# tool-recommender-bot/logparser

Measured on AMD Instinct MI355X. Metric: GB/s (and lines/s) of 'combined' log parsed per GPU and per 8xMI355X node, higher is better.
Workload: dtype u8

## Files before the change

logparser_amd/csrc/kernels_common.h:

```cpp
#pragma once
#include <hip/hip_runtime.h>

#ifndef LP_KERNEL_TU
#define LP_KERNEL_TU 1
#endif

#include <algorithm>

#include "kernels.h"
#include "lp_device.h"

namespace lp {
namespace {

constexpr int CHUNK = 64 * 1024;
constexpr int NL_THREADS = 256;
constexpr int PW = 64;

typedef uint32_t u32x4 __attribute__((ext_vector_type(4)));

__device__ __forceinline__ uint32_t byte_eq(uint32_t w, uint32_t c4) {
    uint32_t x = w ^ c4;
    return ~(((x & 0x7F7F7F7Fu) + 0x7F7F7F7Fu) | x | 0x7F7F7F7Fu);
}
__device__ __forceinline__ uint32_t bits16(uint32_t m0, uint32_t m1, uint32_t m2, uint32_t m3) {
    return bcls::nib(m0) | (bcls::nib(m1) << 4) | (bcls::nib(m2) << 8) | (bcls::nib(m3) << 12);
}

__device__ __forceinline__ uint32_t term_bits(uint4 v, const uint8_t* p, uint64_t pos, uint64_t nbytes) {
    uint32_t lf = bits16(byte_eq(v.x, 0x0A0A0A0Au), byte_eq(v.y, 0x0A0A0A0Au), byte_eq(v.z, 0x0A0A0A0Au),
                         byte_eq(v.w, 0x0A0A0A0Au));
    uint32_t cr = bits16(byte_eq(v.x, 0x0D0D0D0Du), byte_eq(v.y, 0x0D0D0D0Du), byte_eq(v.z, 0x0D0D0D0Du),
                         byte_eq(v.w, 0x0D0D0D0Du));
    if (pos + 16 > nbytes) {
        const uint32_t live = nbytes > pos ? (1u << (uint32_t)(nbytes - pos)) - 1u : 0u;
        lf &= live;
        cr &= live;
    }
    if (cr) {
        uint32_t next_lf = lf >> 1;
        if ((cr & 0x8000u) && pos + 16 < nbytes && p[pos + 16] == '\n') next_lf |= 0x8000u;
        cr &= ~next_lf;
    }
    return lf | cr;
}
__device__ __forceinline__ uint32_t term16(const uint8_t* p, uint64_t pos, uint64_t nbytes) {
    uint4 v = make_uint4(0, 0, 0, 0);
    if (pos + 16 <= nbytes && ((uintptr_t)(p + pos) & 15) == 0) {
        v = *reinterpret_cast<const uint4*>(p + pos);
    } else {
        uint32_t w[4] = {0, 0, 0, 0};
        for (uint64_t k = pos; k < pos + 16 && k < nbytes; ++k) w[(k - pos) >> 2] |= (uint32_t)p[k] << (8 * ((k - pos) & 3));
        v = make_uint4(w[0], w[1], w[2], w[3]);
    }
    return term_bits(v, p, pos, nbytes);
}

__device__ __forceinline__ int lane_id() {
    return (int)__builtin_amdgcn_mbcnt_hi(~0u, __builtin_amdgcn_mbcnt_lo(~0u, 0u));
}

struct WaveStack {
    uint32_t* base;
    __device__ uint32_t& operator[](int k) const { return base[k * PW]; }
};

template <typename LN>
__device__ __forceinline__ LN owner_line(const LN& L, int own) {
    LN R = L;
    R.o = (uint32_t)__shfl((int)L.o, own);
    R.n = __shfl(L.n, own);
    if constexpr (!LN::has_masks)
        R.b = reinterpret_cast<decltype(L.b)>(__shfl((unsigned long long)(uintptr_t)L.b, own));
    return R;
}

struct WaveLines {
    int64_t li0, li, lend;
    bool active;
    uint64_t s, e, w0, w1;
    int n;
};
__device__ __forceinline__ WaveLines wave_lines(const Columns& C, int64_t wave, int64_t n_lines, uint64_t nbytes) {
    WaveLines W;
    W.li0 = wave * PW;
    W.li = W.li0 + (int64_t)lane_id();
    W.active = W.li < n_lines;
    W.lend = W.li0 + PW < n_lines ? W.li0 + PW : n_lines;
    W.s = W.e = 0;
    if (W.active) {
        W.s = C.line_off[W.li];
        W.e = C.line_off[W.li + 1] - 1;
    }
    W.n = (int)((W.e - W.s) > (uint64_t)0x7FFFFFFF ? 0x7FFFFFFF : (W.e - W.s));
    W.w0 = C.line_off[W.li0] & ~15ull;
    W.w1 = C.line_off[W.lend];
    if (W.w1 > nbytes) W.w1 = nbytes;
    return W;
}

__device__ __forceinline__ int crlf_len(int n, uint32_t last) { return n - (n > 0 && last == '\r' ? 1 : 0); }
__device__ __forceinline__ int crlf_len_hbm(const uint8_t* buf, const WaveLines& W) {
    return W.active ? crlf_len(W.n, W.n > 0 ? buf[W.e - 1] : 0u) : W.n;
}

__device__ __forceinline__ bool stage_window(const uint8_t* __restrict__ buf, uint64_t nbytes, uint64_t w0, uint64_t w1,
                                             uint8_t* win, uint16_t* msk16) {
    const int lane = lane_id();
    const int nv = (int)((w1 - w0 + 15) >> 4);
    const int nv4 = (nv + 3) & ~3;
    uint32_t bad = 0;
    constexpr int SB = 20;
    const uint64_t full_end = nbytes & ~15ull;
    for (int k0 = lane; k0 < nv4; k0 += SB * PW) {
        u32x4 v[SB];
#pragma unroll
        for (int j = 0; j < SB; ++j) {
            const int k = k0 + j * PW;
            const uint64_t p = w0 + 16ull * k;
            v[j] = u32x4{0, 0, 0, 0};
            if (k < nv && p + 16 <= full_end) v[j] = __builtin_nontemporal_load(reinterpret_cast<const u32x4*>(buf + p));
        }
#pragma unroll
        for (int j = 0; j < SB; ++j) {
            const int k = k0 + j * PW;
            if (k >= nv4) continue;
            const uint64_t p = w0 + 16ull * k;
            if (k < nv && p + 16 > full_end) {
                auto word = [&](uint64_t q) {
                    uint32_t w = 0;
#pragma unroll
                    for (int b = 0; b < 4; ++b) w |= q + b < nbytes ? (uint32_t)buf[q + b] << (8 * b) : 0u;
                    return w;
                };
                v[j] = u32x4{word(p), word(p + 4), word(p + 8), word(p + 12)};
            }
            *reinterpret_cast<u32x4*>(win + 16 * k) = v[j];
            uint32_t m0, m1, g = 0, lf, other, cr;
            bcls::classify16p(v[j][0], v[j][1], v[j][2], v[j][3], m0, m1, g, lf, other);
            if (other) bcls::classify16c(v[j][0], v[j][1], v[j][2], v[j][3], g, cr);
            if (k < nv) bad |= g;
            msk16[8 * (k >> 2) + (k & 3)] = (uint16_t)m0;
            msk16[8 * (k >> 2) + 4 + (k & 3)] = (uint16_t)m1;
        }
    }
    return !__any(bad != 0);
}

struct WaveCounts {
    uint32_t act = 0, ok = 0, bad = 0, written = 0;
    uint32_t gathered = 0;
    __device__ __forceinline__ void store(LP_G uint32_t* wave_counts, int64_t wave) const {
        if (lane_id() == 0) {
            uint4 c, d;
            c.x = act;
            c.y = ok;
            c.z = bad;
            c.w = act - ok - bad;
            d.x = written;
            d.y = gathered;
            d.z = d.w = 0;
            uint4* wc = reinterpret_cast<uint4*>(wave_counts + WC_WORDS * (size_t)wave);
            wc[0] = c;
            wc[1] = d;
        }
    }
    __device__ __forceinline__ void store(const Columns& C, int64_t wave) const { store(C.wave_counts, wave); }
};

template <bool MULTI, typename LN>
__device__ __forceinline__ void parse_wave(const Program& P, const Elem* elems, const Columns& C, const LN& L,
                                           bool active, int64_t li, WaveStack stk, bool clean, WaveCounts& WC) {
    LineOut o;
    o.status = ST_OK;
    LP_PROF(1);
    if (active) phase1<MULTI>(P, elems, L, o, stk, C, li, clean, P.n_fmt > 1 ? (int)C.fmt_id[li] : 0);
    LP_PROF(9);
    if (active) write_line(P, o, C, li);
    if (active && !P.has_phase2()) C.arena_base[li] = 0;
    WC.act += (uint32_t)__popcll(__ballot(active));
    WC.ok += (uint32_t)__popcll(__ballot(active && o.status == ST_OK));
    WC.bad += (uint32_t)__popcll(__ballot(active && o.status == ST_BAD));
}

__device__ __forceinline__ u32x4 load16(const uint8_t* __restrict__ buf, uint64_t nbytes, uint64_t p) {
    if (p + 16 <= nbytes) return *reinterpret_cast<const u32x4*>(buf + p);
    uint32_t w[4] = {0, 0, 0, 0};
    for (int c = 0; c < 16; ++c) w[c >> 2] |= p + c < nbytes ? (uint32_t)buf[p + c] << (8 * (c & 3)) : 0u;
    return u32x4{w[0], w[1], w[2], w[3]};
}

__device__ __forceinline__ void load_elems(const Program& P, Elem* s_elems) {
    for (int k = lane_id(); k < P.n_elems; k += PW) s_elems[k] = P.elems[k];
}

__device__ __forceinline__ uint32_t select64(uint64_t m, uint32_t k) {
    uint32_t pos = 0, v = (uint32_t)m, c = (uint32_t)__popc(v);
    if (k >= c) { k -= c; v = (uint32_t)(m >> 32); pos = 32; }
    c = (uint32_t)__popc(v & 0xFFFFu);
    if (k >= c) { k -= c; v >>= 16; pos += 16; }
    c = (uint32_t)__popc(v & 0xFFu);
    if (k >= c) { k -= c; v >>= 8; pos += 8; }
    c = (uint32_t)__popc(v & 0xFu);
    if (k >= c) { k -= c; v >>= 4; pos += 4; }
    c = (uint32_t)__popc(v & 3u);
    if (k >= c) { k -= c; v >>= 2; pos += 2; }
    return pos + (k >= (v & 1u) ? 1u : 0u);
}
__device__ __forceinline__ int lsb64(uint64_t m) { return (int)__builtin_ctzll(m); }
__device__ __forceinline__ int msb64(uint64_t m) { return 63 - (int)__builtin_clzll(m); }

template <typename T>
__device__ __forceinline__ T wave_incl_scan(T x) {
    const int lane = lane_id();
    for (int d = 1; d < 64; d <<= 1) {
        const T y = __shfl_up(x, d);
        if (lane >= d) x += y;
    }
    return x;
}
template <typename T>
__device__ __forceinline__ T wave_sum(T x) {
    for (int d = 32; d > 0; d >>= 1) x += __shfl_xor(x, d);
    return x;
}

}
}
```

logparser_amd/csrc/uri.hip:

```cpp
#include "kernels_common.h"

namespace lp {

namespace {

constexpr uint32_t URI_CAP = 8512;
#ifndef LP_URI_QR
#define LP_URI_QR 4
#endif
#ifndef LP_URI_GR
#define LP_URI_GR 9
#endif

template <int NU>
struct UriLane {
    bool ok;
    int fmt;
    uint64_t ls;
    RegArr<NU> sp, cs, usep;
};

template <int NU>
__device__ __forceinline__ UriLane<NU> uri_lane(const Program& P, const Columns& C, int64_t li, bool active) {
    UriLane<NU> U;
    U.sp.fill(0);
    U.cs.fill(0);
    U.usep.fill(0);
    U.ok = false;
    U.fmt = 0;
    U.ls = 0;
    if (!active) return U;
    const uint8_t st = C.status[li];
    const int fmt = P.n_fmt > 1 ? (int)C.fmt_id[li] : 0;
    U.ls = C.line_off[li];
    const uint32_t tf = C.tok_flags[li];
    uint32_t raw[NU], kind[NU];
    for (int u = 0; u < NU; ++u) {
        raw[u] = 0;
        kind[u] = FL_FULL;
        if (u >= P.n_uri || P.uri[u].src_q >= 0) continue;
        if (P.uri[u].src_tok >= 0) {
            raw[u] = C.tok_span[P.uri[u].src_tok][li];
            kind[u] = (tf >> P.uri[u].src_tok) & 1u ? FL_NONE : FL_FULL;
        } else {
            raw[u] = C.fl_uri[P.uri[u].src_fl][li];
            kind[u] = C.fl_kind[P.uri[u].src_fl][li];
        }
    }
    U.ok = st == ST_OK;
    U.fmt = U.ok ? fmt : 0;
    if (U.ok)
        for (int u = 0; u < P.n_uri && u < NU; ++u) {
            const int a = (int)(raw[u] & 0xFFFF), b = (int)(raw[u] >> 16);
            if (P.uri[u].fmt == U.fmt && P.uri[u].src_q < 0 && kind[u] != FL_NONE && b > a) U.sp.set(u, mkspan(a, b));
        }
    return U;
}


template <bool SLOT, typename CL>
__device__ __forceinline__ void uri_walk_coop(const Program& P, int u, const CL& L, bool part, int a, int b,
                                              uint32_t usep, const Arena& A, UriWalk& Wk) {
    const int lane = lane_id();
    const bool table = u >= 0 && P.uri[u].want_query && P.uri[u].query_stage >= 0;
    const uint32_t cnt = part ? usep : 0u;
    uint32_t x = cnt;
    for (int d = 1; d < 64; d <<= 1) {
        const uint32_t y = __shfl_up(x, d);
        if (lane >= d) x += y;
    }
    const uint32_t eb = x - cnt, E = __shfl(x, 63);
    const uint32_t tab = (A.used + 15) & ~15u;
    const unsigned long long reg = (unsigned long long)(uintptr_t)A.p;
    int resume = -1, fa = -1, fpct = -1, lastB = -1, lastPP = -1;
    uint32_t count = 0;
    bool rw = false;
    for (uint32_t g0 = 0; g0 < E; g0 += PW) {
        const uint32_t g = g0 + (uint32_t)lane;
        const bool valid = g < E;
        int ow = 0;
        for (int st = 32; st; st >>= 1)
            if (__shfl((int)eb, ow + st) <= (int)g) ow += st;
        const uint32_t ebo = (uint32_t)__shfl((int)eb, ow);
        const uint32_t oo = (uint32_t)__shfl((int)L.o, ow);
        const int oa = __shfl(a, ow), ob = __shfl(b, ow);
        uint32_t Aq = 0;
        if (valid) {
            const uint32_t A0 = oo + (uint32_t)oa, A1 = oo + (uint32_t)ob, WL = (A1 - 1) >> 6;
            uint32_t W = A0 >> 6, k = g - ebo;
            uint64_t m = L.mask(MC_UEV, W) & (~0ull << (A0 & 63));
            for (;;) {
                if (W == WL) m &= ~0ull >> (63 - ((A1 - 1) & 63));
                const uint32_t c = (uint32_t)__popcll(m);
                if (k < c || W >= WL) break;
                k -= c;
                ++W;
                m = L.mask(MC_UEV, W);
            }
            Aq = (W << 6) + select64(m, k);
        }
        const int q = (int)(Aq - oo);
        CL Lo = L;
        Lo.o = oo;
        Lo.n = ob;
        const uint32_t w = valid ? load_u32_at(Lo, q) : 0u;
        const uint32_t c = w & 0xFFu;
        const bool pct = c == '%';
        const bool bad_pct = pct && (q + 2 >= ob || !is_hex((w >> 8) & 0xFFu) || !is_hex((w >> 16) & 0xFFu));
        const bool stop = valid && (c == '#' || c == ';' || c >= 0x80 || bad_pct);
        const bool aq = c == '&' || c == '?';
        const int cres = __shfl(resume, ow), cfa = __shfl(fa, ow), clB = __shfl(lastB, ow), clPP = __shfl(lastPP, ow);
        const uint32_t ccount = (uint32_t)__shfl((int)count, ow);
        const int s0 = (int)ebo - (int)g0;
        const uint64_t below = (1ull << lane) - 1ull;
        const uint64_t seg_lt = valid ? below & (~0ull << (s0 > 0 ? s0 : 0)) : 0ull;
        const uint64_t Bstop = __ballot(stop);
        const bool live = valid && !stop && cres < 0 && !(Bstop & seg_lt);
        const uint64_t Baq = __ballot(live && aq);
        const uint64_t mfa = Baq & seg_lt;
        const int qfa = __shfl(q, mfa ? lsb64(mfa) : lane);
        const int fa_j = cfa >= 0 ? cfa : (mfa ? qfa : -1);
        const bool pp = live && ((pct && !bad_pct) || c == '+');
        const bool otable = SLOT ? __shfl((int)table, ow) != 0 : table;
        const bool isB = otable && live && aq && fa_j >= 0;
        const uint64_t BB = __ballot(isB), BPP = __ballot(pp);
        const uint64_t mB = BB & seg_lt, mP = BPP & seg_lt;
        const int qpb = __shfl(q, mB ? msb64(mB) : lane), qpp = __shfl(q, mP ? msb64(mP) : lane);
        const bool first_piece = !mB && clB < 0;
        const int pb = mB ? qpb : (clB >= 0 ? clB : fa_j);
        const int lpp = mP ? qpp : clPP;
        const int lp = first_piece ? lpp : (lpp > pb ? lpp : -1);
        const bool emit = isB && q > pb + 1;
        const uint64_t BE = __ballot(emit);
        const bool rwj = live && fa_j >= 0 && ((aq && c == '?') || (!aq && !pct && uri_needs_encode(c)));
        const uint64_t BR = __ballot(rwj);
        const unsigned long long oreg = __shfl(reg, ow);
        const uint32_t otab = (uint32_t)__shfl((int)tab, ow);
        if (emit) {
            const uint32_t idx = ccount + (uint32_t)__popcll(BE & seg_lt);
            const uint64_t t0 = (uint64_t)(uint32_t)(pb + 1) | ((uint64_t)(uint32_t)q << 16) | ((uint64_t)(uint32_t)(lp + 1) << 48);
            *reinterpret_cast<LP_G u32x4*>(reinterpret_cast<LP_G uint8_t*>(oreg) + otab + 16 * idx) =
                u32x4{(uint32_t)t0, (uint32_t)(t0 >> 32), 0u, 0u};
        }
        const int so = (int)eb - (int)g0, eo = (int)(eb + cnt) - (int)g0;
        const int so_c = so < 0 ? 0 : so > PW ? PW : so, eo_c = eo < 0 ? 0 : eo > PW ? PW : eo;
        const uint64_t segm = so_c < eo_c ? ((eo_c == PW ? ~0ull : (1ull << eo_c) - 1ull) & (~0ull << so_c)) : 0ull;
        const uint64_t ms = Bstop & segm, mf = Baq & segm, mpct = __ballot(live && pct) & segm, mb = BB & segm,
                       mpp = BPP & segm;
        const int q_s = __shfl(q, ms ? lsb64(ms) : lane), q_f = __shfl(q, mf ? lsb64(mf) : lane);
        const int q_p = __shfl(q, mpct ? lsb64(mpct) : lane), q_b = __shfl(q, mb ? msb64(mb) : lane);
        const int q_pp = __shfl(q, mpp ? msb64(mpp) : lane);
        if (resume < 0 && ms) resume = q_s;
        if (fa < 0 && mf) fa = q_f;
        if (fpct < 0 && mpct) fpct = q_p;
        if (mb) lastB = q_b;
        if (mpp) lastPP = q_pp;
        count += (uint32_t)__popcll(BE & segm);
        rw = rw || (BR & segm) != 0;
    }
    if (!part) return;
    Wk.resume = resume;
    Wk.fa = fa;
    Wk.first_pct = fpct;
    Wk.rewr = rw ? 2u : 0u;
    QueryTable& T = Wk.T;
    if (table && fa >= 0) {
        T.on = T.set = true;
        T.maxp = usep + 1;
        T.tab = tab;
        T.reg = tab + 16 * T.maxp;
        T.s = (lastB >= 0 ? lastB : fa) + 1;
        T.count = count;
        T.lp = lastB >= 0 ? (lastPP > lastB ? lastPP : -1) : lastPP;
    } else {
        T.lp = lastPP;
    }
}

template <int NU, int NQ, bool COOP, bool SLOT, bool QUEUE, typename LU, typename LL>
__device__ __forceinline__ void uri_wave(const Program& P, const Columns& C, UriLane<NU>& U, LU&& lu, LL&& ll,
                                         bool active, int64_t li, int64_t wave, WaveCounts& WC, bool& redo) {
    const int lane = lane_id();
    const int nq = P.n_query < NQ ? P.n_query : NQ;
    uint32_t need = 0;
    if (U.ok)
        for (int u = 0; u < P.n_uri && u < NU; ++u) {
            const uint32_t s = U.sp.get(u);
            if (!s) continue;
            uint32_t ev;
            need += uri_need(P, u, lu(u), (int)(s & 0xFFFF), (int)(s >> 16), ev);
            U.usep.set(u, ev);
        }
    int lend = 0;
    if (U.ok) {
        for (int j = 0; j < P.n_list; ++j)
            if (P.list[j].fmt == U.fmt) lend = max(lend, (int)(C.tok_span[P.list[j].tok][li] >> 16));
        for (int j = 0; j < P.n_pair; ++j)
            if (P.pair[j].fmt == U.fmt) lend = max(lend, (int)(C.tok_span[P.pair[j].tok][li] >> 16));
    }
    if (lend) ll(lend, [&](const auto& LH) { need += list_need(P, U.fmt, LH, C, li) + pair_need(P, U.fmt, LH, C, li); });
    need = (need + 15) & ~15u;
    uint32_t x = need;
    for (int d = 1; d < 64; d <<= 1) {
        uint32_t y = __shfl_up(x, d);
        if (lane >= d) x += y;
    }
    const uint32_t total = __shfl(x, 63);
    const int shard = (int)(wave % ARENA_SHARDS);
    unsigned long long wbase = 0;
    if (lane == 63 && total) wbase = atomicAdd(&C.meta->shard_top[16 * shard], (unsigned long long)total + 12ull);
    wbase = (__shfl(wbase, 63) + 15) & ~15ull;
    const bool fits = wbase + total <= C.shard_cap;
    LP_PROF(26);
    uint32_t written = 0;
    unsigned long long my_region = 0;
    UriOutT<NQ> o;
    o.qlist.fill(0);
    o.qpend.fill(0);
    o.status = U.ok ? ST_OK : ST_BAD;
    Arena A{C.arena, 0, 0};
    bool live = false;
    if (U.ok) {
        if (!fits && need) {
            o.status = ST_FALLBACK;
            atomicAdd(&C.meta->arena_ovf, 1ull);
        } else {
            const unsigned long long mine = (unsigned long long)shard * C.shard_cap + wbase + x - need;
            my_region = mine;
            C.arena_base[li] = mine;
            A = Arena{C.arena + mine, 0, need};
            A.top = &C.meta->shard_top[16 * shard];
            A.base = wbase + x - need;
            A.limit = C.shard_cap;
            live = true;
        }
    }
    const int nu = P.n_uri < NU ? P.n_uri : NU;
    for (int sl = 0; sl < nu; ++sl) {
        int u = sl;
        if constexpr (SLOT) {
            u = -1;
            for (int v = 0, c = 0; v < nu; ++v)
                if (P.uri[v].fmt == U.fmt) {
                    if (c == sl) u = v;
                    ++c;
                }
            if (!__any(u >= 0)) break;
        }
        const bool fmt_ok = live && o.status == ST_OK && u >= 0 && P.uri[u].fmt == U.fmt;
        const uint32_t sp = U.sp.get(u);
        const int a = (int)(sp & 0xFFFF), b = (int)(sp >> 16);
        const bool part = fmt_ok && b > a;
        if (fmt_ok && !part) {
            C.u_flags[u][li] = 0;
            if (P.uri[u].query_stage >= 0) { C.q_count[P.uri[u].query_stage][li] = 0; C.q_params[P.uri[u].query_stage][li] = 0; }
        }
        LP_PROF(10 + 2 * sl);
        UriWalk Wk;
        if constexpr (COOP) {
            LP_PROF(50 + 4 * sl);
            uri_walk_coop<SLOT>(P, u, lu(u), part, a, b, U.usep.get(u), A, Wk);
            LP_PROF(51 + 4 * sl);
        } else if (part) {
            uri_walk_fast(P, u, lu(u), a, b, U.usep.get(u), A, Wk);
        }
        if (part) {
            const int st = uri_stage_rest<UR_OFF>(P, u, lu(u), a, b, U.usep.get(u), A, C, li, o, Wk);
            if (st != ST_OK) o.status = st;
        }
        LP_PROF(11 + 2 * sl);
    }
    if (live && lend && o.status == ST_OK) {
        bool filled = true;
        ll(lend, [&](const auto& LH) { filled = list_fill(P, U.fmt, LH, A, C, li) && pair_fill(P, U.fmt, LH, A, C, li); });
        if (!filled) o.status = ST_FALLBACK;
    }
    if (live) {
        if (A.ovf) {
            o.status = ST_FALLBACK;
            atomicAdd(&C.meta->arena_ovf, 1ull);
        }
        written = A.used - A.slack + A.extra;
    }
    LP_PROF(21);
    if (nq > 0) {
        constexpr int QR = LP_URI_QR;
        __syncthreads();
        const bool has = U.ok && o.status == ST_OK && need != 0;
        const unsigned long long my_ab = has ? my_region : 0ull;
        uint64_t piece_ovf = 0;
        uint32_t np = 0;
        for (int qs = 0; qs < nq; ++qs) np += has ? o.qpend.get(qs) : 0u;
        uint32_t incl = np;
        for (int d = 1; d < 64; d <<= 1) {
            const uint32_t y = __shfl_up(incl, d);
            if (lane >= d) incl += y;
        }
        const uint32_t base = incl - np, tot = __shfl(incl, 63);
        auto piece = [&](int ow, uint32_t j, int& pq, uint32_t& soff) {
            uint32_t cum = 0;
            pq = 0;
            soff = 0;
            for (int qs = 0; qs < nq; ++qs) {
                const uint32_t c = (uint32_t)__shfl((int)(has ? o.qpend.get(qs) : 0u), ow);
                const uint32_t l = (uint32_t)__shfl((int)o.qlist.get(qs), ow);
                if (j >= cum && j < cum + c) {
                    pq = qs;
                    soff = l + 16 * (j - cum);
                }
                cum += c;
            }
        };
        auto owner_view = [&](int ow, int pq) {
            auto OL = owner_line(lu(P.query[0].uri), ow);
            for (int qs = 1; qs < nq; ++qs) {
                const auto V = owner_line(lu(P.query[qs].uri), ow);
                if (pq == qs) OL = V;
            }
            return OL;
        };
        for (uint32_t g0 = 0; g0 < tot; g0 += QR * PW) {
            int own[QR], pqs[QR];
            uint32_t soffs[QR];
            uint64_t t0[QR];
#pragma unroll
            for (int k = 0; k < QR; ++k) {
                own[k] = 0;
                pqs[k] = 0;
                soffs[k] = 0;
                t0[k] = 0;
                if (g0 + (uint32_t)(k * PW) >= tot) continue;
                const uint32_t g = g0 + (uint32_t)(k * PW + lane);
                int ow = 0;
                for (int st = 32; st; st >>= 1)
                    if (__shfl(base, ow + st) <= g) ow += st;
                own[k] = ow;
                const uint32_t ob = __shfl(base, ow);
                const unsigned long long oab = __shfl(my_ab, ow);
                piece(ow, g - ob, pqs[k], soffs[k]);
                if (g < tot) t0[k] = *reinterpret_cast<const LP_G uint64_t*>(C.arena + oab + soffs[k]);
            }
            LP_PROF(17);
            QPrep qp[QR];
            uint32_t mine = 0;
#pragma unroll
            for (int k = 0; k < QR; ++k) {
                if (g0 + (uint32_t)(k * PW) >= tot) continue;
                const uint32_t g = g0 + (uint32_t)(k * PW + lane);
                const auto OL = owner_view(own[k], pqs[k]);
                if (g < tot) qp[k] = query_prep(OL, t0[k]);
                mine += qp[k].need;
            }
            LP_PROF(18);
            uint32_t x = mine;
            for (int d = 1; d < 64; d <<= 1) {
                const uint32_t y = __shfl_up(x, d);
                if (lane >= d) x += y;
            }
            const uint32_t rtot = __shfl(x, 63);
            unsigned long long rbase = 0;
            if (lane == 63 && rtot) rbase = atomicAdd(&C.meta->shard_top[16 * shard], (unsigned long long)rtot);
            unsigned long long at = __shfl(rbase, 63) + x - mine;
            LP_PROF(19);
#pragma unroll
            for (int k = 0; k < QR; ++k) {
                if (g0 + (uint32_t)(k * PW) >= tot) continue;
                const uint32_t g = g0 + (uint32_t)(k * PW + lane);
                const int ow = own[k];
                const unsigned long long oab = __shfl(my_ab, ow);
                const auto OL = owner_view(ow, pqs[k]);
                bool povf = false;
                if (g < tot) {
                    LP_G uint64_t* slot = reinterpret_cast<LP_G uint64_t*>(C.arena + oab + soffs[k]);
                    const unsigned long long rel = oab - (unsigned long long)shard * C.shard_cap;
                    if (qp[k].need && (at + qp[k].need > C.shard_cap || at - rel + qp[k].need > 0x7FFFFFFFull)) {
                        slot[0] = REF_SKIP;
                        slot[1] = 0;
                        povf = true;
                        atomicAdd(&C.meta->arena_ovf, 1ull);
                    } else {
                        Arena A{C.arena + oab, (uint32_t)(at - rel), (uint32_t)(at - rel + qp[k].need)};
                        written += query_finish(P, P.query[pqs[k]], OL, A, C.arena + oab, slot, qp[k]);
                    }
                    at += qp[k].need;
                }
                for (uint64_t m = __ballot(povf); m; m &= m - 1) piece_ovf |= 1ull << __shfl(ow, (int)__builtin_ctzll(m));
            }
        }
        if (((piece_ovf >> lane) & 1) && o.status == ST_OK) o.status = ST_FALLBACK;
    }
    LP_PROF(22);
    redo = false;
    if (U.ok && o.status == ST_REPAIR) {
        o.status = ST_FALLBACK;
        if constexpr (QUEUE) {
            const unsigned long long k = atomicAdd(&C.meta->uri_fix_lines, 1ull);
            if (k < (unsigned long long)C.cap_lines) C.uri_fix_list[k] = (uint32_t)li;
        } else {
            redo = true;
        }
    }
    if (U.ok && o.status != ST_OK) C.status[li] = (uint8_t)o.status;
    for (int d = 32; d > 0; d >>= 1) written += __shfl_xor(written, d);
    const int st = !active ? -1 : U.ok ? o.status : (int)C.status[li];
    WC.act += (uint32_t)__popcll(__ballot(active));
    WC.ok += (uint32_t)__popcll(__ballot(st == ST_OK));
    WC.bad += (uint32_t)__popcll(__ballot(st == ST_BAD));
    WC.written += written;
}


template <int NU, int NQ, bool SLOT, uint32_t CAP>
__device__ __forceinline__ bool uri_compact(const uint8_t* __restrict__ buf, uint64_t nbytes, const Program& P,
                                            const Columns& C, int64_t wave, int64_t n_lines, uint32_t* cbuf,
                                            uint64_t* plane, WaveCounts& WC, bool& redo) {
    const int lane = lane_id();
    const int64_t li = wave * PW + lane;
    const bool active = li < n_lines;
    LP_PROF(23);
    UriLane<NU> U = uri_lane<NU>(P, C, li, active);
    LP_PROF(27);
    uint64_t lo = ~0ull, hi = 0;
    for (int u = 0; u < P.n_uri && u < NU; ++u) {
        const uint32_t s = U.sp.get(u);
        if (!s) continue;
        lo = min(lo, U.ls + (s & 0xFFFF));
        hi = max(hi, U.ls + (s >> 16));
    }
    const uint64_t r0 = hi ? lo & ~15ull : 0;
    const uint32_t nb1 = hi ? (uint32_t)((((hi + 15) & ~15ull) - r0) >> 4) : 0u;
    const bool lists = P.n_list > 0 || P.n_pair > 0;
    uint64_t l0 = ~0ull, l1 = 0;
    if (lists && U.ok) {
        auto add = [&](int tok) {
            const uint32_t s = C.tok_span[tok][li];
            if ((s >> 16) > (s & 0xFFFFu)) {
                l0 = min(l0, U.ls + (s & 0xFFFFu));
                l1 = max(l1, U.ls + (s >> 16));
            }
        };
        for (int j = 0; j < P.n_list; ++j)
            if (P.list[j].fmt == U.fmt) add(P.list[j].tok);
        for (int j = 0; j < P.n_pair; ++j)
            if (P.pair[j].fmt == U.fmt) add(P.pair[j].tok);
    }
    const uint64_t q0 = l1 ? l0 & ~15ull : 0;
    const uint32_t nb2 = l1 ? (uint32_t)((((l1 + 15) & ~15ull) - q0) >> 4) : 0u;
    auto blocks = [&](uint32_t n, uint32_t& first) {
        uint32_t x = n;
        for (int d = 1; d < 64; d <<= 1) {
            const uint32_t y = __shfl_up(x, d);
            if (lane >= d) x += y;
        }
        first = x - n;
        return (uint32_t)__shfl(x, 63);
    };
    uint32_t cb;
    uint32_t tot = blocks(nb1 + nb2, cb);
    bool lin = lists;
    if (lists && 16 * tot + 16 > CAP) {
        lin = false;
        tot = blocks(nb1, cb);
    }
    if (16 * tot + 16 > CAP) return false;
    WC.gathered = 16 * tot;
    for (int u = 0; u < P.n_uri && u < NU; ++u) {
        const uint32_t s = U.sp.get(u);
        if (s) U.cs.set(u, 16 * cb + (uint32_t)(U.ls + (s & 0xFFFF) - r0));
    }
    constexpr int GR = LP_URI_GR;
    uint16_t* pl16 = reinterpret_cast<uint16_t*>(plane);
    for (uint32_t g0 = 0; g0 < tot; g0 += GR * PW) {
        u32x4 v[GR];
#pragma unroll
        for (int k = 0; k < GR; ++k) {
            const uint32_t g = g0 + (uint32_t)(k * PW + lane);
            int own = 0;
            for (int st = 32; st; st >>= 1)
                if (__shfl(cb, own + st) <= g) own += st;
            const uint32_t j = g - (uint32_t)__shfl(cb, own);
            uint64_t src = (uint64_t)__shfl((unsigned long long)r0, own) + 16ull * j;
            if (lin) {
                const uint32_t n1 = (uint32_t)__shfl(nb1, own);
                const uint64_t s1 = (uint64_t)__shfl((unsigned long long)q0, own);
                if (j >= n1) src = s1 + 16ull * (j - n1);
            }
            v[k] = u32x4{0, 0, 0, 0};
            if (g < tot) v[k] = load16(buf, nbytes, src);
        }
        LP_PROF(28);
#pragma unroll
        for (int k = 0; k < GR; ++k) {
            const uint32_t g = g0 + (uint32_t)(k * PW + lane);
            if (g >= tot) continue;
            *reinterpret_cast<u32x4*>(cbuf + 4 * g) = v[k];
            pl16[g] = (uint16_t)bcls::classify16u(v[k][0], v[k][1], v[k][2], v[k][3]);
        }
    }
    LP_PROF(24);
    for (uint32_t g = tot + lane; g < ((tot + 1 + 3) & ~3u); g += PW) {
        *reinterpret_cast<u32x4*>(cbuf + 4 * g) = u32x4{0, 0, 0, 0};
        pl16[g] = 0;
    }
    __syncthreads();
    LP_PROF(25);
    typedef LineT<lds_bytes, lds_u64, 1> CL;
    auto lu = [&](int u) {
        const uint32_t s = U.sp.get(u);
        return CL{(lds_bytes)cbuf, U.cs.get(u) - (s & 0xFFFFu), (int)(s >> 16), (lds_u64)plane};
    };
    const LP_G uint8_t* lsp = (const LP_G uint8_t*)buf + U.ls;
    const uint32_t lmis = (uint32_t)((uintptr_t)lsp & 3);
    const uint32_t lorig = 16 * (cb + nb1) + (uint32_t)(U.ls - q0);
    auto ll = [&](int lend, auto&& f) {
        if (lin) f(LineT<lds_bytes>{(lds_bytes)cbuf, lorig, lend});
        else f(LineT<const LP_G uint8_t*>{lsp - lmis, lmis, lend});
    };
    uri_wave<NU, NQ, true, SLOT, CAP == URI_CAP>(P, C, U, lu, ll, active, li, wave, WC, redo);
    return true;
}

#ifndef LP_URI_SLOT_WPE
#define LP_URI_SLOT_WPE 4
#endif
template <int NU, int NQ, bool SLOT>
__global__ __launch_bounds__(PW, SLOT ? LP_URI_SLOT_WPE : 4) void k_uri_lines(const uint8_t* __restrict__ buf, uint64_t nbytes,
                                                     const DeviceArgs* __restrict__ args) {
    const Program& P = args->prog;
    const Columns& C = args->cols;
    const int64_t n_lines = (int64_t)C.meta->n_lines;
    const int64_t wave = blockIdx.x;
    if (wave * PW >= n_lines || C.meta->cap_ovf) return;
    __shared__ __attribute__((aligned(16))) uint32_t cbuf[URI_CAP / 4 + 16];
    __shared__ uint64_t plane[URI_CAP / 64 + 1];
    WaveCounts WC;
    bool redo;
    if (uri_compact<NU, NQ, SLOT, URI_CAP>(buf, nbytes, P, C, wave, n_lines, cbuf, plane, WC, redo)) WC.store(C, wave);
    else if (lane_id() == 0) C.uri_ovf_list[atomicAdd(&C.meta->uri_ovf_waves, 1ull)] = (uint32_t)wave;
}

__device__ __forceinline__ void uri_redo_line(const uint8_t* __restrict__ buf, uint64_t nbytes, const Program& P,
                                              const Columns& C, int64_t n_lines, int64_t li) {
    if ((uint64_t)li >= (uint64_t)n_lines) return;
    const uint64_t s = C.line_off[li], e = C.line_off[li + 1] - 1;
    if (e < s || e - s > 0xFFFFull || e > nbytes) return;
    const int n = crlf_len((int)(e - s), e > s ? buf[e - 1] : 0u);
    const LP_G uint8_t* ls = (const LP_G uint8_t*)(buf) + s;
    const uint32_t mis = (uint32_t)((uintptr_t)ls & 3);
    const LineT<const LP_G uint8_t*> L{ls - mis, mis, n};
    const int fmt = P.n_fmt > 1 ? (int)C.fmt_id[li] : 0;
    RegArr<MAX_URI> sp, usep;
    sp.fill(0);
    usep.fill(0);
    uint32_t need = 0;
    for (int u = 0; u < P.n_uri; ++u) {
        int a, b;
        if (P.uri[u].fmt != fmt || !uri_source_cols(P, C, li, u, a, b) || b > n) continue;
        uint32_t ev;
        need += uri_need(P, u, L, a, b, ev);
        sp.set(u, mkspan((uint32_t)a, (uint32_t)b));
        usep.set(u, ev);
    }
    need += list_need(P, fmt, L, C, li) + pair_need(P, fmt, L, C, li);
    need = (need + 15) & ~15u;
    const int shard = (int)((li / PW) % ARENA_SHARDS);
    LP_G unsigned long long* top = &C.meta->shard_top[16 * shard];
    const unsigned long long x = (atomicAdd(top, (unsigned long long)need + 12ull) + 15) & ~15ull;
    int st = ST_FALLBACK;
    uint32_t written = 0;
    if (x + need > C.shard_cap) {
        atomicAdd(&C.meta->arena_ovf, 1ull);
    } else {
        const unsigned long long mine = (unsigned long long)shard * C.shard_cap + x;
        C.arena_base[li] = mine;
        Arena A{C.arena + mine, 0, need};
        A.top = top;
        A.base = x;
        A.limit = C.shard_cap;
        UriOut o;
        o.qlist.fill(0);
        o.qpend.fill(0);
        auto lu = [&](int) { return L; };
        phase2<UR_ON>(P, fmt, lu, sp, usep, o, A, C, li);
        if (o.status == ST_OK) query_pieces_serial(P, lu, o, A);
        if (o.status == ST_OK && (!list_fill(P, fmt, L, A, C, li) || !pair_fill(P, fmt, L, A, C, li))) o.status = ST_FALLBACK;
        if (A.ovf) {
            o.status = ST_FALLBACK;
            atomicAdd(&C.meta->arena_ovf, 1ull);
        }
        st = o.status;
        written = A.used - A.slack + A.extra;
    }
    LP_G uint32_t* wc = C.wave_counts + WC_WORDS * (size_t)(li / PW);
    if (st != ST_FALLBACK) {
        C.status[li] = (uint8_t)st;
        atomicAdd(&wc[st == ST_OK ? 1 : 2], 1u);
        atomicSub(&wc[3], 1u);
    }
    if (written) atomicAdd(&wc[4], written);
}

constexpr uint32_t URI_CAP_OVF = 4 * URI_CAP;
template <int NU, int NQ, bool SLOT>
__global__ __launch_bounds__(PW) void k_uri_overflow(const uint8_t* __restrict__ buf, uint64_t nbytes,
                                                     const DeviceArgs* __restrict__ args) {
    const Program& P = args->prog;
    const Columns& C = args->cols;
    const int64_t n_lines = (int64_t)C.meta->n_lines;
    const uint64_t nq = C.meta->uri_ovf_waves;
    const uint64_t nfix = min((uint64_t)(uint32_t)C.meta->uri_fix_lines, (uint64_t)C.cap_lines);
    __shared__ __attribute__((aligned(16))) uint32_t cbuf[URI_CAP_OVF / 4 + 16];
    __shared__ uint64_t plane[URI_CAP_OVF / 64 + 1];
    for (uint64_t q = blockIdx.x; q < nq; q += gridDim.x) {
        const int64_t wave = C.uri_ovf_list[q];
        WaveCounts WC;
        bool redo = false;
        if (!uri_compact<NU, NQ, SLOT, URI_CAP_OVF>(buf, nbytes, P, C, wave, n_lines, cbuf, plane, WC, redo)) {
            const WaveLines W = wave_lines(C, wave, n_lines, nbytes);
            UriLane<NU> U = uri_lane<NU>(P, C, W.li, W.active);
            const LP_G uint8_t* ls = (const LP_G uint8_t*)(buf) + W.s;
            const uint32_t mis = (uint32_t)((uintptr_t)ls & 3);
            const LineT<const LP_G uint8_t*> L{ls - mis, mis, crlf_len_hbm(buf, W)};
            auto lu = [&](int) { return L; };
            auto ll = [&](int lend, auto&& f) { f(LineT<const LP_G uint8_t*>{ls - mis, mis, lend}); };
            uri_wave<NU, NQ, false, SLOT, false>(P, C, U, lu, ll, W.active, W.li, wave, WC, redo);
        }
        __syncthreads();
        WC.store(C, wave);
        if (__any(redo)) {
            __threadfence();
            if (redo) {
                atomicAdd(&C.meta->uri_fix_lines, 1ull << 32);
                uri_redo_line(buf, nbytes, P, C, n_lines, wave * PW + lane_id());
            }
        }
    }
    for (uint64_t q = (uint64_t)blockIdx.x * PW + (uint64_t)lane_id(); q < nfix; q += (uint64_t)gridDim.x * PW)
        uri_redo_line(buf, nbytes, P, C, n_lines, (int64_t)C.uri_fix_list[q]);
}

__global__ __launch_bounds__(PW) void k_derived_lines(const uint8_t* __restrict__ buf, uint64_t nbytes,
                                                      const DeviceArgs* __restrict__ args) {
    const Program& P = args->prog;
    const Columns& C = args->cols;
    const int64_t n_lines = (int64_t)C.meta->n_lines;
    const int64_t wave = blockIdx.x;
    if (wave * PW >= n_lines || C.meta->cap_ovf) return;
    const WaveLines W = wave_lines(C, wave, n_lines, nbytes);
    int st = W.active ? (int)C.status[W.li] : -1;
    if (st == ST_OK) {
        const int fmt = P.n_fmt > 1 ? (int)C.fmt_id[W.li] : 0;
        const LP_G uint8_t* ls = (const LP_G uint8_t*)(buf) + W.s;
        const uint32_t mis = (uint32_t)((uintptr_t)ls & 3);
        const unsigned long long ab = C.arena_base[W.li];
        const int shard = (int)(ab / C.shard_cap);
        Arena R{C.arena + ab, 0, 0};
        R.top = &C.meta->shard_top[16 * shard];
        R.base = ab - (unsigned long long)shard * C.shard_cap;
        R.limit = C.shard_cap;
        st = derived_line(P, fmt, ls - mis, mis, crlf_len_hbm(buf, W), R, C, W.li);
        if (R.ovf) atomicAdd(&C.meta->arena_ovf, 1ull);
        if (st != ST_OK) C.status[W.li] = (uint8_t)st;
    }
    const uint32_t ok = (uint32_t)__popcll(__ballot(st == ST_OK)), bad = (uint32_t)__popcll(__ballot(st == ST_BAD));
    if (lane_id() == 0) {
        LP_G uint32_t* wc = C.wave_counts + WC_WORDS * (size_t)wave;
        const uint32_t act = wc[0];
        wc[1] = ok;
        wc[2] = bad;
        wc[3] = act - ok - bad;
    }
}

}

int launch_uri(const ParseLaunch& a, const DeviceArgs* d_args, hipStream_t s) {
    const int64_t waves = parse_waves(a.cap_lines);
    if (waves == 0 || !a.uri) return 0;
    const int64_t grid = waves < 1024 ? waves : 1024;
    if (!a.chunked) {
        hipLaunchKernelGGL((k_uri_lines<MAX_URI, MAX_QUERY, true>), dim3((unsigned)waves), dim3(PW), 0, s, a.buf,
                           a.nbytes, d_args);
        hipLaunchKernelGGL((k_uri_overflow<MAX_URI, MAX_QUERY, true>), dim3((unsigned)grid), dim3(PW), 0, s, a.buf,
                           a.nbytes, d_args);
    } else if (a.n_uri <= 2 && a.n_query <= 2) {
        hipLaunchKernelGGL((k_uri_lines<2, 2, false>), dim3((unsigned)waves), dim3(PW), 0, s, a.buf, a.nbytes, d_args);
        hipLaunchKernelGGL((k_uri_overflow<2, 2, false>), dim3((unsigned)grid), dim3(PW), 0, s, a.buf, a.nbytes, d_args);
    } else {
        hipLaunchKernelGGL((k_uri_lines<MAX_URI, MAX_QUERY, false>), dim3((unsigned)waves), dim3(PW), 0, s, a.buf,
                           a.nbytes, d_args);
        hipLaunchKernelGGL((k_uri_overflow<MAX_URI, MAX_QUERY, false>), dim3((unsigned)grid), dim3(PW), 0, s, a.buf,
                           a.nbytes, d_args);
    }
    if (a.derived) hipLaunchKernelGGL(k_derived_lines, dim3((unsigned)waves), dim3(PW), 0, s, a.buf, a.nbytes, d_args);
    return hipGetLastError() == hipSuccess ? 0 : -1;
}

#if defined(LP_PROFILE)
int prof_read_uri(unsigned long long* out) {
    return hipMemcpyFromSymbol(out, HIP_SYMBOL(g_prof), sizeof(unsigned long long) * PROF_WAVES * PROF_POINTS) == hipSuccess ? 0 : -1;
}
int prof_clear_uri() {
    static unsigned long long z[PROF_WAVES * PROF_POINTS];
    return hipMemcpyToSymbol(HIP_SYMBOL(g_prof), z, sizeof z) == hipSuccess ? 0 : -1;
}
#endif

}
```

Measured before the change: 660.2.

## Replace shuffle binary-search owner lookup with LDS head bitmap and DPP scans

Swaps the wave-wide Hillis-Steele shuffle prefix scans for DPP-based inclusive scans with readlane totals. Replaces the per-item 6-step shuffle binary search that finds each gathered item's owning lane with an LDS bitmap of segment heads plus a rank table, resolved by popcount/select. The aim is to cut cross-lane shuffle traffic in the URI compaction and query-piece loops, at the price of extra LDS storage, atomics and __syncthreads per round. Trailing zero-work rounds are now skipped.

```diff
diff --git a/logparser_amd/csrc/kernels_common.h b/logparser_amd/csrc/kernels_common.h
--- a/logparser_amd/csrc/kernels_common.h
+++ b/logparser_amd/csrc/kernels_common.h
@@ -9,6 +9,7 @@
 
 #include "kernels.h"
 #include "lp_device.h"
+#include "lp_owner.h"
 
 namespace lp {
 namespace {
@@ -194,19 +195,6 @@
     for (int k = lane_id(); k < P.n_elems; k += PW) s_elems[k] = P.elems[k];
 }
 
-__device__ __forceinline__ uint32_t select64(uint64_t m, uint32_t k) {
-    uint32_t pos = 0, v = (uint32_t)m, c = (uint32_t)__popc(v);
-    if (k >= c) { k -= c; v = (uint32_t)(m >> 32); pos = 32; }
-    c = (uint32_t)__popc(v & 0xFFFFu);
-    if (k >= c) { k -= c; v >>= 16; pos += 16; }
-    c = (uint32_t)__popc(v & 0xFFu);
-    if (k >= c) { k -= c; v >>= 8; pos += 8; }
-    c = (uint32_t)__popc(v & 0xFu);
-    if (k >= c) { k -= c; v >>= 4; pos += 4; }
-    c = (uint32_t)__popc(v & 3u);
-    if (k >= c) { k -= c; v >>= 2; pos += 2; }
-    return pos + (k >= (v & 1u) ? 1u : 0u);
-}
 __device__ __forceinline__ int lsb64(uint64_t m) { return (int)__builtin_ctzll(m); }
 __device__ __forceinline__ int msb64(uint64_t m) { return 63 - (int)__builtin_clzll(m); }
 
@@ -219,6 +207,19 @@
     }
     return x;
 }
+__device__ __forceinline__ uint32_t wave_incl_scan_dpp(uint32_t x) {
+    constexpr int ROW_SHR = 0x110, ROW_BCAST15 = 0x142, ROW_BCAST31 = 0x143;
+    x += (uint32_t)__builtin_amdgcn_update_dpp(0, (int)x, ROW_SHR + 1, 0xF, 0xF, false);
+    x += (uint32_t)__builtin_amdgcn_update_dpp(0, (int)x, ROW_SHR + 2, 0xF, 0xF, false);
+    x += (uint32_t)__builtin_amdgcn_update_dpp(0, (int)x, ROW_SHR + 4, 0xF, 0xF, false);
+    x += (uint32_t)__builtin_amdgcn_update_dpp(0, (int)x, ROW_SHR + 8, 0xF, 0xF, false);
+    x += (uint32_t)__builtin_amdgcn_update_dpp(0, (int)x, ROW_BCAST15, 0xA, 0xF, false);
+    x += (uint32_t)__builtin_amdgcn_update_dpp(0, (int)x, ROW_BCAST31, 0xC, 0xF, false);
+    return x;
+}
+__device__ __forceinline__ uint32_t lane_value(uint32_t x, int l) {
+    return (uint32_t)__builtin_amdgcn_readlane((int)x, l);
+}
 template <typename T>
 __device__ __forceinline__ T wave_sum(T x) {
     for (int d = 32; d > 0; d >>= 1) x += __shfl_xor(x, d);
diff --git a/logparser_amd/csrc/lp_owner.h b/logparser_amd/csrc/lp_owner.h
--- /dev/null
+++ b/logparser_amd/csrc/lp_owner.h
@@ -0,0 +1,40 @@
+#pragma once
+#include <stdint.h>
+
+#if !defined(__HIP__)
+#ifndef __host__
+#define __host__
+#endif
+#ifndef __device__
+#define __device__
+#endif
+#endif
+
+namespace lp {
+
+__host__ __device__ inline uint32_t select64(uint64_t m, uint32_t k) {
+    uint32_t pos = 0, v = (uint32_t)m, c = (uint32_t)__builtin_popcount(v);
+    if (k >= c) { k -= c; v = (uint32_t)(m >> 32); pos = 32; }
+    c = (uint32_t)__builtin_popcount(v & 0xFFFFu);
+    if (k >= c) { k -= c; v >>= 16; pos += 16; }
+    c = (uint32_t)__builtin_popcount(v & 0xFFu);
+    if (k >= c) { k -= c; v >>= 8; pos += 8; }
+    c = (uint32_t)__builtin_popcount(v & 0xFu);
+    if (k >= c) { k -= c; v >>= 4; pos += 4; }
+    c = (uint32_t)__builtin_popcount(v & 3u);
+    if (k >= c) { k -= c; v >>= 2; pos += 2; }
+    return pos + (k >= (v & 1u) ? 1u : 0u);
+}
+
+__host__ __device__ inline uint64_t owner_heads_upto(uint64_t H, int i) { return H & ((2ull << i) - 1ull); }
+
+__host__ __device__ inline uint32_t owner_rank(uint32_t K, uint64_t H, int i) {
+    return K + (uint32_t)__builtin_popcountll(owner_heads_upto(H, i));
+}
+
+__host__ __device__ inline int owner_lane(uint64_t N, uint32_t K, uint64_t H, int i) {
+    const uint32_t rank = owner_rank(K, H, i);
+    return rank ? (int)(select64(N, rank - 1) & 63u) : 0;
+}
+
+}
diff --git a/logparser_amd/csrc/uri.hip b/logparser_amd/csrc/uri.hip
--- a/logparser_amd/csrc/uri.hip
+++ b/logparser_amd/csrc/uri.hip
@@ -11,6 +11,43 @@
 #ifndef LP_URI_GR
 #define LP_URI_GR 9
 #endif
+
+constexpr int OWNER_WORDS = LP_URI_GR;
+constexpr int OWNER_LDS_WORDS = OWNER_WORDS + PW / 2;
+struct OwnerRounds {
+    uint64_t* hw;
+    uint32_t* tab;
+    uint32_t first;
+    bool has;
+    uint32_t b0;
+
+    __device__ __forceinline__ OwnerRounds(uint64_t* words, uint32_t first_item, uint32_t cnt)
+        : hw(words), tab(reinterpret_cast<uint32_t*>(words + OWNER_WORDS)), first(first_item), has(cnt != 0), b0(0) {
+        const uint64_t N = __ballot(has);
+        const uint32_t r = __builtin_amdgcn_mbcnt_hi((uint32_t)(N >> 32), __builtin_amdgcn_mbcnt_lo((uint32_t)N, 0u));
+        __syncthreads();
+        if (has) tab[r] = (uint32_t)lane_id() | first << 6;
+    }
+    __device__ __forceinline__ void fill(uint32_t from) {
+        b0 = from;
+        __syncthreads();
+        if (lane_id() < OWNER_WORDS) hw[lane_id()] = 0;
+        __syncthreads();
+        const uint32_t r = (first - from) >> 6;
+        if (has && first >= from && r < (uint32_t)OWNER_WORDS)
+            atomicOr(reinterpret_cast<unsigned long long*>(hw + r), 1ull << (first & 63u));
+        __syncthreads();
+    }
+    __device__ __forceinline__ void fill_at(uint32_t g0) {
+        if ((g0 >> 6) % (uint32_t)OWNER_WORDS == 0) fill(g0);
+    }
+    __device__ __forceinline__ int owner(uint32_t g0, uint32_t& ofirst) const {
+        const uint32_t K = (uint32_t)__popcll(__ballot(has && first < g0));
+        const uint32_t e = tab[owner_rank(K, hw[(g0 - b0) >> 6], lane_id()) - 1u];
+        ofirst = e >> 6;
+        return (int)(e & 63u);
+    }
+};
 
 template <int NU>
 struct UriLane {
@@ -60,16 +97,13 @@
 
 template <bool SLOT, typename CL>
 __device__ __forceinline__ void uri_walk_coop(const Program& P, int u, const CL& L, bool part, int a, int b,
-                                              uint32_t usep, const Arena& A, UriWalk& Wk) {
+                                              uint32_t usep, const Arena& A, uint64_t* heads, UriWalk& Wk) {
     const int lane = lane_id();
     const bool table = u >= 0 && P.uri[u].want_query && P.uri[u].query_stage >= 0;
     const uint32_t cnt = part ? usep : 0u;
-    uint32_t x = cnt;
-    for (int d = 1; d < 64; d <<= 1) {
-        const uint32_t y = __shfl_up(x, d);
-        if (lane >= d) x += y;
-    }
-    const uint32_t eb = x - cnt, E = __shfl(x, 63);
+    const uint32_t x = wave_incl_scan_dpp(cnt);
+    const uint32_t eb = x - cnt, E = lane_value(x, 63);
+    OwnerRounds OW(heads, eb, cnt);
     const uint32_t tab = (A.used + 15) & ~15u;
     const unsigned long long reg = (unsigned long long)(uintptr_t)A.p;
     int resume = -1, fa = -1, fpct = -1, lastB = -1, lastPP = -1;
@@ -78,10 +112,9 @@
     for (uint32_t g0 = 0; g0 < E; g0 += PW) {
         const uint32_t g = g0 + (uint32_t)lane;
         const bool valid = g < E;
-        int ow = 0;
-        for (int st = 32; st; st >>= 1)
-            if (__shfl((int)eb, ow + st) <= (int)g) ow += st;
-        const uint32_t ebo = (uint32_t)__shfl((int)eb, ow);
+        OW.fill_at(g0);
+        uint32_t ebo;
+        const int ow = OW.owner(g0, ebo);
         const uint32_t oo = (uint32_t)__shfl((int)L.o, ow);
         const int oa = __shfl(a, ow), ob = __shfl(b, ow);
         uint32_t Aq = 0;
@@ -179,7 +212,8 @@
 
 template <int NU, int NQ, bool COOP, bool SLOT, bool QUEUE, typename LU, typename LL>
 __device__ __forceinline__ void uri_wave(const Program& P, const Columns& C, UriLane<NU>& U, LU&& lu, LL&& ll,
-                                         bool active, int64_t li, int64_t wave, WaveCounts& WC, bool& redo) {
+                                         bool active, int64_t li, int64_t wave, uint64_t* heads, WaveCounts& WC,
+                                         bool& redo) {
     const int lane = lane_id();
     const int nq = P.n_query < NQ ? P.n_query : NQ;
     uint32_t need = 0;
@@ -200,12 +234,10 @@
     }
     if (lend) ll(lend, [&](const auto& LH) { need += list_need(P, U.fmt, LH, C, li) + pair_need(P, U.fmt, LH, C, li); });
     need = (need + 15) & ~15u;
-    uint32_t x = need;
-    for (int d = 1; d < 64; d <<= 1) {
-        uint32_t y = __shfl_up(x, d);
-        if (lane >= d) x += y;
-    }
-    const uint32_t total = __shfl(x, 63);
+    LP_PROF(29);
+    const uint32_t x = wave_incl_scan_dpp(need);
+    const uint32_t total = lane_value(x, 63);
+    LP_PROF(20);
     const int shard = (int)(wave % ARENA_SHARDS);
     unsigned long long wbase = 0;
     if (lane == 63 && total) wbase = atomicAdd(&C.meta->shard_top[16 * shard], (unsigned long long)total + 12ull);
@@ -259,7 +291,7 @@
         UriWalk Wk;
         if constexpr (COOP) {
             LP_PROF(50 + 4 * sl);
-            uri_walk_coop<SLOT>(P, u, lu(u), part, a, b, U.usep.get(u), A, Wk);
+            uri_walk_coop<SLOT>(P, u, lu(u), part, a, b, U.usep.get(u), A, heads, Wk);
             LP_PROF(51 + 4 * sl);
         } else if (part) {
             uri_walk_fast(P, u, lu(u), a, b, U.usep.get(u), A, Wk);
@@ -291,12 +323,9 @@
         uint64_t piece_ovf = 0;
         uint32_t np = 0;
         for (int qs = 0; qs < nq; ++qs) np += has ? o.qpend.get(qs) : 0u;
-        uint32_t incl = np;
-        for (int d = 1; d < 64; d <<= 1) {
-            const uint32_t y = __shfl_up(incl, d);
-            if (lane >= d) incl += y;
-        }
-        const uint32_t base = incl - np, tot = __shfl(incl, 63);
+        const uint32_t incl = wave_incl_scan_dpp(np);
+        const uint32_t base = incl - np, tot = lane_value(incl, 63);
+        OwnerRounds OW(heads, base, np);
         auto piece = [&](int ow, uint32_t j, int& pq, uint32_t& soff) {
             uint32_t cum = 0;
             pq = 0;
@@ -331,11 +360,10 @@
                 t0[k] = 0;
                 if (g0 + (uint32_t)(k * PW) >= tot) continue;
                 const uint32_t g = g0 + (uint32_t)(k * PW + lane);
-                int ow = 0;
-                for (int st = 32; st; st >>= 1)
-                    if (__shfl(base, ow + st) <= g) ow += st;
+                OW.fill_at(g0 + (uint32_t)(k * PW));
+                uint32_t ob;
+                const int ow = OW.owner(g0 + (uint32_t)(k * PW), ob);
                 own[k] = ow;
-                const uint32_t ob = __shfl(base, ow);
                 const unsigned long long oab = __shfl(my_ab, ow);
                 piece(ow, g - ob, pqs[k], soffs[k]);
                 if (g < tot) t0[k] = *reinterpret_cast<const LP_G uint64_t*>(C.arena + oab + soffs[k]);
@@ -352,12 +380,8 @@
                 mine += qp[k].need;
             }
             LP_PROF(18);
-            uint32_t x = mine;
-            for (int d = 1; d < 64; d <<= 1) {
-                const uint32_t y = __shfl_up(x, d);
-                if (lane >= d) x += y;
-            }
-            const uint32_t rtot = __shfl(x, 63);
+            const uint32_t x = wave_incl_scan_dpp(mine);
+            const uint32_t rtot = lane_value(x, 63);
             unsigned long long rbase = 0;
             if (lane == 63 && rtot) rbase = atomicAdd(&C.meta->shard_top[16 * shard], (unsigned long long)rtot);
             unsigned long long at = __shfl(rbase, 63) + x - mine;
@@ -413,7 +437,7 @@
 template <int NU, int NQ, bool SLOT, uint32_t CAP>
 __device__ __forceinline__ bool uri_compact(const uint8_t* __restrict__ buf, uint64_t nbytes, const Program& P,
                                             const Columns& C, int64_t wave, int64_t n_lines, uint32_t* cbuf,
-                                            uint64_t* plane, WaveCounts& WC, bool& redo) {
+                                            uint64_t* plane, uint64_t* heads, WaveCounts& WC, bool& redo) {
     const int lane = lane_id();
     const int64_t li = wave * PW + lane;
     const bool active = li < n_lines;
@@ -447,20 +471,17 @@
     const uint64_t q0 = l1 ? l0 & ~15ull : 0;
     const uint32_t nb2 = l1 ? (uint32_t)((((l1 + 15) & ~15ull) - q0) >> 4) : 0u;
     auto blocks = [&](uint32_t n, uint32_t& first) {
-        uint32_t x = n;
-        for (int d = 1; d < 64; d <<= 1) {
-            const uint32_t y = __shfl_up(x, d);
-            if (lane >= d) x += y;
-        }
+        const uint32_t x = wave_incl_scan_dpp(n);
         first = x - n;
-        return (uint32_t)__shfl(x, 63);
+        return lane_value(x, 63);
     };
-    uint32_t cb;
-    uint32_t tot = blocks(nb1 + nb2, cb);
+    uint32_t cb, nb = nb1 + nb2;
+    uint32_t tot = blocks(nb, cb);
     bool lin = lists;
     if (lists && 16 * tot + 16 > CAP) {
         lin = false;
-        tot = blocks(nb1, cb);
+        nb = nb1;
+        tot = blocks(nb, cb);
     }
     if (16 * tot + 16 > CAP) return false;
     WC.gathered = 16 * tot;
@@ -470,22 +491,24 @@
     }
     constexpr int GR = LP_URI_GR;
     uint16_t* pl16 = reinterpret_cast<uint16_t*>(plane);
+    OwnerRounds OW(heads, cb, nb);
     for (uint32_t g0 = 0; g0 < tot; g0 += GR * PW) {
         u32x4 v[GR];
+        OW.fill(g0);
 #pragma unroll
         for (int k = 0; k < GR; ++k) {
+            v[k] = u32x4{0, 0, 0, 0};
+            if (g0 + (uint32_t)(k * PW) >= tot) continue;
             const uint32_t g = g0 + (uint32_t)(k * PW + lane);
-            int own = 0;
-            for (int st = 32; st; st >>= 1)
-                if (__shfl(cb, own + st) <= g) own += st;
-            const uint32_t j = g - (uint32_t)__shfl(cb, own);
+            uint32_t ocb;
+            const int own = OW.owner(g0 + (uint32_t)(k * PW), ocb);
+            const uint32_t j = g - ocb;
             uint64_t src = (uint64_t)__shfl((unsigned long long)r0, own) + 16ull * j;
             if (lin) {
                 const uint32_t n1 = (uint32_t)__shfl(nb1, own);
                 const uint64_t s1 = (uint64_t)__shfl((unsigned long long)q0, own);
                 if (j >= n1) src = s1 + 16ull * (j - n1);
             }
-            v[k] = u32x4{0, 0, 0, 0};
             if (g < tot) v[k] = load16(buf, nbytes, src);
         }
         LP_PROF(28);
@@ -516,7 +539,7 @@
         if (lin) f(LineT<lds_bytes>{(lds_bytes)cbuf, lorig, lend});
         else f(LineT<const LP_G uint8_t*>{lsp - lmis, lmis, lend});
     };
-    uri_wave<NU, NQ, true, SLOT, CAP == URI_CAP>(P, C, U, lu, ll, active, li, wave, WC, redo);
+    uri_wave<NU, NQ, true, SLOT, CAP == URI_CAP>(P, C, U, lu, ll, active, li, wave, heads, WC, redo);
     return true;
 }
 
@@ -533,9 +556,10 @@
     if (wave * PW >= n_lines || C.meta->cap_ovf) return;
     __shared__ __attribute__((aligned(16))) uint32_t cbuf[URI_CAP / 4 + 16];
     __shared__ uint64_t plane[URI_CAP / 64 + 1];
+    __shared__ uint64_t heads[OWNER_LDS_WORDS];
     WaveCounts WC;
     bool redo;
-    if (uri_compact<NU, NQ, SLOT, URI_CAP>(buf, nbytes, P, C, wave, n_lines, cbuf, plane, WC, redo)) WC.store(C, wave);
+    if (uri_compact<NU, NQ, SLOT, URI_CAP>(buf, nbytes, P, C, wave, n_lines, cbuf, plane, heads, WC, redo)) WC.store(C, wave);
     else if (lane_id() == 0) C.uri_ovf_list[atomicAdd(&C.meta->uri_ovf_waves, 1ull)] = (uint32_t)wave;
 }
 
@@ -611,11 +635,12 @@
     const uint64_t nfix = min((uint64_t)(uint32_t)C.meta->uri_fix_lines, (uint64_t)C.cap_lines);
     __shared__ __attribute__((aligned(16))) uint32_t cbuf[URI_CAP_OVF / 4 + 16];
     __shared__ uint64_t plane[URI_CAP_OVF / 64 + 1];
+    __shared__ uint64_t heads[OWNER_LDS_WORDS];
     for (uint64_t q = blockIdx.x; q < nq; q += gridDim.x) {
         const int64_t wave = C.uri_ovf_list[q];
         WaveCounts WC;
         bool redo = false;
-        if (!uri_compact<NU, NQ, SLOT, URI_CAP_OVF>(buf, nbytes, P, C, wave, n_lines, cbuf, plane, WC, redo)) {
+        if (!uri_compact<NU, NQ, SLOT, URI_CAP_OVF>(buf, nbytes, P, C, wave, n_lines, cbuf, plane, heads, WC, redo)) {
             const WaveLines W = wave_lines(C, wave, n_lines, nbytes);
             UriLane<NU> U = uri_lane<NU>(P, C, W.li, W.active);
             const LP_G uint8_t* ls = (const LP_G uint8_t*)(buf) + W.s;
@@ -623,7 +648,7 @@
             const LineT<const LP_G uint8_t*> L{ls - mis, mis, crlf_len_hbm(buf, W)};
             auto lu = [&](int) { return L; };
             auto ll = [&](int lend, auto&& f) { f(LineT<const LP_G uint8_t*>{ls - mis, mis, lend}); };
-            uri_wave<NU, NQ, false, SLOT, false>(P, C, U, lu, ll, W.active, W.li, wave, WC, redo);
+            uri_wave<NU, NQ, false, SLOT, false>(P, C, U, lu, ll, W.active, W.li, wave, heads, WC, redo);
         }
         __syncthreads();
         WC.store(C, wave);
```

Result: faster. 687.3 (median of 6 runs) (+4.1%).
